# myshell-ai/OpenVoice

Measured on AMD Instinct MI355X. Metric: real_time_factor, higher is better.
Workload: dtype f32; 1 GPU; ToneColorConverter.convert path, 32 x 10 s @ 22.05 kHz per GPU (T=861 frames), fp32, calibrated random weights; batch_per_gpu=32, global_batch=32, parallelism=dp1 (utterance sharding, RCCL broadcast of src/tgt se)

## Files before the change

include/openvoice_amd.h:

```cpp
#ifndef OPENVOICE_AMD_H
#define OPENVOICE_AMD_H

#include <stddef.h>
#include <stdint.h>

#ifdef __cplusplus
extern "C" {
#endif

typedef void* ov_stream_t;

enum {
  OV_OK = 0,
  OV_E_BADARG = -1,
  OV_E_UNSUPPORTED = -2,
  OV_E_ALIGN = -3,
  OV_E_LAUNCH = -4
};

enum {
  OV_EPI_LINEAR = 0,
  OV_EPI_GATE = 1,
  OV_EPI_RESSKIP = 2,
  OV_EPI_COUPLE = 3,
// ... 309 lines not shown
  const float* bias;
  float* out;
  const float* res;
  const float* add;
  int64_t x_bstride, out_bstride, res_bstride, add_bstride;
  int32_t B, Cin, Cout, L;
  int32_t x_ld, out_ld;
  int32_t K, dil;
  int32_t nwg;
  int32_t frags;
  float in_slope;
  float scale;
  unsigned long long* dbg;
  const int32_t* col_limit;
  int32_t col_limit_scale;
  float out_slope;
} ov_conv1d_wino_params;
int ov_conv1d_wino_f32(const ov_conv1d_wino_params* p, ov_stream_t stream);
int ov_conv1d_wino_supported(int Cin, int Cout, int K, int dil);
int ov_conv1d_wino_chunk(int K, int Cout);
size_t ov_conv1d_wino_pack_size(int Cout, int Cin, int K);
int ov_conv1d_wino_pack_f32(const float* w, int Cout, int Cin, int K, float* dst);

int ov_version(void);
#define OV_ABI_VERSION 212
int ov_build_experiment(void);

#ifdef __cplusplus
}
#endif
#endif
```

openvoice_amd/_lib.py:

```python
import ctypes
import os

_HERE = os.path.dirname(os.path.abspath(__file__))
LIB_PATH = os.environ.get("OPENVOICE_AMD_LIB") or os.path.join(_HERE, "libopenvoice_amd.so")

OV_OK = 0
MIN_VERSION = 212
OV_ERRORS = {-1: "OV_E_BADARG", -2: "OV_E_UNSUPPORTED", -3: "OV_E_ALIGN", -4: "OV_E_LAUNCH"}

EPI_LINEAR, EPI_GATE, EPI_RESSKIP, EPI_COUPLE, EPI_POSTERIOR, EPI_CONVT, EPI_MAGNITUDE = range(7)
F_MASK_V = 1
F_OUT2_INIT = 2
F_CONVT_GROUPED = 4
F_NO_XCD_MAP = 8

_fp = ctypes.c_void_p
_i = ctypes.c_int
_i64 = ctypes.c_int64
LN_PRE_RELU, LN_POST_GELU = 1, 2


class ConvParams(ctypes.Structure):
    _fields_ = [
        ("x", _fp), ("w", _fp), ("bias", _fp), ("bias_b", _fp), ("out", _fp), ("res", _fp),
# ... 60 lines not shown
                ("nwg", ctypes.c_int32), ("frags", ctypes.c_int32),
                ("in_slope", ctypes.c_float), ("scale", ctypes.c_float), ("dbg", _fp),
                ("col_limit", _fp), ("col_limit_scale", ctypes.c_int32), ("out_slope", ctypes.c_float)]


class WnLayerParams(ctypes.Structure):
    _fields_ = [("x", _fp), ("out", _fp), ("skip", _fp), ("w_in", _fp), ("b_in", _fp), ("cond", _fp), ("w_rs", _fp),
                ("b_rs", _fp), ("mask", _fp),
                ("bstride", ctypes.c_int64), ("cond_bstride", ctypes.c_int64), ("mask_bstride", ctypes.c_int64),
                ("B", ctypes.c_int32), ("H", ctypes.c_int32), ("T", ctypes.c_int32), ("ld", ctypes.c_int32),
                ("K", ctypes.c_int32), ("first", ctypes.c_int32), ("last", ctypes.c_int32), ("width", ctypes.c_int32),
                ("ntile", ctypes.c_int32), ("row_split", ctypes.c_int32), ("dbg", _fp), ("acts", _fp)]


SIGNATURES = {
    "ov_version": (ctypes.c_int, []),
    "ov_build_experiment": (ctypes.c_int, []),
    "ov_conv1d_pack_size": (ctypes.c_size_t, [ctypes.c_int, ctypes.c_int, ctypes.c_int]),
    "ov_conv1d_pack_rows": (ctypes.c_int, [ctypes.c_int]),
    "ov_conv1d_pack_f32": (ctypes.c_int, [_fp, ctypes.c_int, ctypes.c_int, ctypes.c_int, _fp]),
    "ov_conv1d_f32": (ctypes.c_int, [ctypes.POINTER(ConvParams), _fp]),
    "ov_resblock_pair_f32": (ctypes.c_int, [ctypes.POINTER(RespairParams), _fp]),
    "ov_resblock_pair_supported": (ctypes.c_int, [_i, _i, _i]),
    "ov_wn_layer_f32": (ctypes.c_int, [ctypes.POINTER(WnLayerParams), _fp]),
    "ov_wn_layer_supported": (ctypes.c_int, [_i, _i]),
    "ov_wn_pack_size": (ctypes.c_size_t, [_i, _i, _i]),
    "ov_wn_pack_f32": (ctypes.c_int, [_fp, _i, _i, _i, _fp]),
    "ov_wn_layer_tile": (ctypes.c_int, [_i, _i, _i]),
    "ov_wn_layer_wino_f32": (ctypes.c_int, [ctypes.POINTER(WnLayerParams), _fp]),
    "ov_wn_layer_wino_tile": (ctypes.c_int, []),
    "ov_wn_wino_pack_size": (ctypes.c_size_t, [_i, _i, _i]),
    "ov_wn_wino_pack_f32": (ctypes.c_int, [_fp, _i, _i, _i, _fp]),
    "ov_conv_post_tanh_f32": (ctypes.c_int, [_fp, _fp, _fp, ctypes.c_int, ctypes.c_int, ctypes.c_int,
                                             ctypes.c_int, ctypes.c_float, _fp]),
    "ov_conv_post_tanh_limited_f32": (ctypes.c_int, [_fp, _fp, _fp, ctypes.c_int, ctypes.c_int, ctypes.c_int,
                                                     ctypes.c_int, ctypes.c_float, _fp, ctypes.c_int, _fp]),
    "ov_frame_limits_i32": (ctypes.c_int, [_fp, _fp, _i, _i, _i, _fp]),
    "ov_linear_f32": (ctypes.c_int, [_fp, _fp, _fp, _fp, ctypes.c_int, ctypes.c_int, ctypes.c_int, _fp]),
    "ov_sequence_mask_f32": (ctypes.c_int, [_fp, _fp, ctypes.c_int, ctypes.c_int, ctypes.c_int, _fp]),
    "ov_unpad_rows_f32": (ctypes.c_int, [_fp, _fp, ctypes.c_int, ctypes.c_int, ctypes.c_int, _fp]),
    "ov_polyphase_fir_f32": (ctypes.c_int, [_fp, _fp, _fp, ctypes.c_int64, ctypes.c_int64, _i, _i, _i, _fp]),
    "ov_polyphase_fir_rows_f32": (ctypes.c_int, [_fp, _i, _fp, _i64, _fp, _i64, _fp, _i64, _i64, _fp]),
    "ov_layernorm_freq_f32": (ctypes.c_int, [_fp, _fp, _fp, _fp, ctypes.c_int, ctypes.c_int, ctypes.c_int,
                                             ctypes.c_float, _fp]),
    "ov_conv2d_s2_relu_f32": (ctypes.c_int, [_fp, _fp, _fp, _fp, ctypes.c_int, ctypes.c_int, ctypes.c_int,
                                             ctypes.c_int, ctypes.c_int, _fp]),
# ... 83 lines not shown
    return _lib


def torch_op(name, *args):
    try:
        return getattr(torch_ops(), name)(*args)
    except RuntimeError as exc:
        if isinstance(exc, OvError):
            raise
        raise OvError(str(exc).split("\n")[0]) from None


def check(code, what):
    if code != OV_OK:
        raise OvError(f"{what} failed: {OV_ERRORS.get(code, code)}")


SHIM_PATH = os.path.join(_HERE, "libopenvoice_amd_torch.so")
_ops = None
VALUE_FUNCS = {"ov_version", "ov_build_experiment", "ov_conv1d_pack_size", "ov_conv1d_pack_rows", "ov_wn_pack_size",
               "ov_conv1d_bf16_pack_size", "ov_resblock_pair_supported", "ov_wn_layer_supported", "ov_wn_layer_tile",
               "ov_resblock_pair_bf16_supported", "ov_resblock_pair2_bf16_supported", "ov_conv1d_split3_pack_size",
               "ov_conv1d_split3_supported", "ov_conv1d_wino_supported", "ov_conv1d_wino_chunk", "ov_conv1d_wino_pack_size",
               "ov_wn_layer_wino_tile", "ov_wn_wino_pack_size"}


def binding():
    b = os.environ.get("OPENVOICE_AMD_BINDING", "ctypes" if os.environ.get("OPENVOICE_AMD_LIB") else "torch")
    if b not in ("torch", "ctypes"):
        raise OvError(f"OPENVOICE_AMD_BINDING={b!r}: expected 'torch' or 'ctypes'")
    return b


def use_torch_binding():
    return binding() == "torch"


def torch_ops():
    global _ops
    if _ops is None:
        import torch
        for path in (LIB_PATH, SHIM_PATH):
            if not os.path.exists(path):
                raise OvError(f"{path} not found: build the HIP extension first (python -c 'import __graft_entry__ "
                              f"as g; g.build()'); there is no CPU fallback (OPENVOICE_AMD_BINDING=ctypes needs only "
                              f"libopenvoice_amd.so)")
        torch.ops.load_library(SHIM_PATH)
# ... 49 lines not shown
```

openvoice_amd/csrc/torch_shim.cpp:

```cpp
#include <ATen/ATen.h>
#include <ATen/hip/impl/HIPGuardImplMasqueradingAsCUDA.h>
#include <c10/hip/HIPStream.h>
#include <torch/library.h>

#include <string>
#include <type_traits>

#include "openvoice_amd.h"

namespace {

const char* ov_strerror(int rc) {
  switch (rc) {
    case OV_E_BADARG: return "OV_E_BADARG";
    case OV_E_UNSUPPORTED: return "OV_E_UNSUPPORTED";
    case OV_E_ALIGN: return "OV_E_ALIGN";
    case OV_E_LAUNCH: return "OV_E_LAUNCH";
    default: return "unknown error";
  }
}

using OptTensor = c10::optional<at::Tensor>;

struct Ctx {
// ... 180 lines not shown
  DeviceScope scope(c);
  finish(ov_conv1d_f32(&p, c.stream()), "ov_conv1d_f32");
}

void resblock_pair_f32(const OptTensor& x, const OptTensor& w1, const OptTensor& b1, const OptTensor& w2,
                       const OptTensor& b2, const OptTensor& out, const OptTensor& add, const OptTensor& dbg,
                       const OptTensor& col_limit, at::IntArrayRef ip, at::ArrayRef<double> fp) {
  TORCH_CHECK(ip.size() == 11 && fp.size() == 2, "openvoice_amd::resblock_pair_f32: 11 integer and 2 float parameters");
  Ctx c{"resblock_pair_f32", false};
  ov_respair_params p{};
  p.x = sptr<float>(x, c, 0); p.w1 = sptr<float>(w1, c, 1); p.b1 = sptr<float>(b1, c, 2);
  p.w2 = sptr<float>(w2, c, 3); p.b2 = sptr<float>(b2, c, 4); p.out = sptr<float>(out, c, 5);
  p.add = sptr<float>(add, c, 6);
  p.dbg = sptr<unsigned long long>(dbg, c, 7);
  p.col_limit = sptr<int32_t>(col_limit, c, 8);
  p.B = (int32_t)ip[0]; p.C = (int32_t)ip[1]; p.L = (int32_t)ip[2]; p.ld = (int32_t)ip[3]; p.K = (int32_t)ip[4];
  p.dil = (int32_t)ip[5]; p.nwg = (int32_t)ip[6];
  p.x_bstride = ip[7]; p.out_bstride = ip[8]; p.add_bstride = ip[9]; p.col_limit_scale = (int32_t)ip[10];
  p.slope = (float)fp[0]; p.scale = (float)fp[1];
  DeviceScope scope(c);
  finish(ov_resblock_pair_f32(&p, c.stream()), "ov_resblock_pair_f32");
}

template <int (*FN)(const ov_wn_layer_params*, ov_stream_t)>
void wn_layer_any(const char* op, const char* entry, const OptTensor& x, const OptTensor& out, const OptTensor& skip,
                  const OptTensor& w_in, const OptTensor& b_in, const OptTensor& cond, const OptTensor& w_rs,
                  const OptTensor& b_rs, const OptTensor& mask, const OptTensor& dbg, const OptTensor& acts,
                  at::IntArrayRef ip) {
  TORCH_CHECK(ip.size() == 13, "openvoice_amd::", op, ": 13 integer parameters");
  Ctx c{op, false};
  ov_wn_layer_params p{};
  p.x = sptr<float>(x, c, 0); p.out = sptr<float>(out, c, 1); p.skip = sptr<float>(skip, c, 2);
  p.w_in = sptr<float>(w_in, c, 3); p.b_in = sptr<float>(b_in, c, 4); p.cond = sptr<float>(cond, c, 5, ip[11]);
  p.w_rs = sptr<float>(w_rs, c, 6); p.b_rs = sptr<float>(b_rs, c, 7); p.mask = sptr<float>(mask, c, 8);
  p.dbg = sptr<unsigned long long>(dbg, c, 9);
  p.acts = sptr<float>(acts, c, 10);
  p.B = (int32_t)ip[0]; p.H = (int32_t)ip[1]; p.T = (int32_t)ip[2]; p.ld = (int32_t)ip[3]; p.K = (int32_t)ip[4];
  p.first = (int32_t)ip[5]; p.last = (int32_t)ip[6]; p.width = (int32_t)ip[7];
  p.bstride = ip[8]; p.cond_bstride = ip[9]; p.mask_bstride = ip[10]; p.row_split = (int32_t)ip[12];
  DeviceScope scope(c);
  finish(FN(&p, c.stream()), entry);
}
void wn_layer_f32(const OptTensor& x, const OptTensor& out, const OptTensor& skip, const OptTensor& w_in,
                  const OptTensor& b_in, const OptTensor& cond, const OptTensor& w_rs, const OptTensor& b_rs,
                  const OptTensor& mask, const OptTensor& dbg, const OptTensor& acts, at::IntArrayRef ip) {
  wn_layer_any<&ov_wn_layer_f32>("wn_layer_f32", "ov_wn_layer_f32", x, out, skip, w_in, b_in, cond, w_rs, b_rs, mask, dbg, acts, ip);
// ... 77 lines not shown
                     at::ArrayRef<double> fp) {
  TORCH_CHECK(ip.size() == 15 && fp.size() == 3, "openvoice_amd::conv1d_wino_f32: 15 integer and 3 float parameters");
  Ctx c{"conv1d_wino_f32", false};
  ov_conv1d_wino_params p{};
  p.x = sptr<float>(x, c, 0); p.w = sptr<float>(w, c, 1); p.bias = sptr<float>(bias, c, 2);
  p.out = sptr<float>(out, c, 3); p.res = sptr<float>(res, c, 4); p.add = sptr<float>(add, c, 5);
  p.dbg = sptr<unsigned long long>(dbg, c, 6);
  p.col_limit = sptr<int32_t>(col_limit, c, 7); p.col_limit_scale = (int32_t)ip[14];
  p.B = (int32_t)ip[0]; p.Cin = (int32_t)ip[1]; p.Cout = (int32_t)ip[2]; p.L = (int32_t)ip[3];
  p.x_ld = (int32_t)ip[4]; p.out_ld = (int32_t)ip[5]; p.K = (int32_t)ip[6]; p.dil = (int32_t)ip[7]; p.nwg = (int32_t)ip[8];
  p.x_bstride = ip[9]; p.out_bstride = ip[10]; p.res_bstride = ip[11]; p.add_bstride = ip[12]; p.frags = (int32_t)ip[13];
  p.in_slope = (float)fp[0]; p.scale = (float)fp[1]; p.out_slope = (float)fp[2];
  DeviceScope scope(c);
  finish(ov_conv1d_wino_f32(&p, c.stream()), "ov_conv1d_wino_f32");
}

}

TORCH_LIBRARY(openvoice_amd, m) {
  m.def("conv1d_f32(Tensor? x, Tensor? w, Tensor? bias, Tensor(a!)? out, Tensor? res, Tensor? add, Tensor(b!)? out2, "
        "Tensor? mask, Tensor? bias_b, Tensor? col_limit, int[] ip, float[] fp) -> ()", &conv1d_f32);
  m.def("resblock_pair_f32(Tensor? x, Tensor? w1, Tensor? b1, Tensor? w2, Tensor? b2, Tensor(a!)? out, Tensor? add, "
        "Tensor(b!)? dbg, Tensor? col_limit, int[] ip, float[] fp) -> ()", &resblock_pair_f32);
  m.def("wn_layer_f32(Tensor? x, Tensor(a!)? out, Tensor(b!)? skip, Tensor? w_in, Tensor? b_in, Tensor? cond, Tensor? w_rs, "
        "Tensor? b_rs, Tensor? mask, Tensor(c!)? dbg, Tensor(d!)? acts, int[] ip) -> ()", &wn_layer_f32);
  m.def("wn_layer_wino_f32(Tensor? x, Tensor(a!)? out, Tensor(b!)? skip, Tensor? w_in, Tensor? b_in, Tensor? cond, Tensor? w_rs, "
        "Tensor? b_rs, Tensor? mask, Tensor(c!)? dbg, Tensor(d!)? acts, int[] ip) -> ()", &wn_layer_wino_f32);
  m.def("conv1d_bf16cl(Tensor? x, Tensor? w, Tensor? bias, Tensor(a!)? out, Tensor? res, Tensor? add, Tensor(b!)? dbg, "
        "int[] ip, float[] fp) -> ()", &conv1d_bf16cl);
  m.def("resblock_pair_bf16cl(Tensor? x, Tensor? w1, Tensor? b1, Tensor? w2, Tensor? b2, Tensor(a!)? out, Tensor? add, "
        "Tensor(b!)? dbg, int[] ip, float[] fp) -> ()", &resblock_pair_bf16cl);
  m.def("resblock_pair2_bf16cl(Tensor? x, Tensor? w1, Tensor? b1, Tensor? w2, Tensor? b2, Tensor(a!)? out, Tensor? add, "
        "Tensor(b!)? dbg, int[] ip, float[] fp) -> ()", &resblock_pair2_bf16cl);
  m.def("conv1d_split3(Tensor? x, Tensor? w, Tensor? bias, Tensor(a!)? out, Tensor? res, Tensor(b!)? dbg, "
        "Tensor? col_limit, int[] ip, float[] fp) -> ()", &conv1d_split3);
  m.def("conv1d_wino_f32(Tensor? x, Tensor? w, Tensor? bias, Tensor(a!)? out, Tensor? res, Tensor? add, Tensor(b!)? dbg, "
        "Tensor? col_limit, int[] ip, float[] fp) -> ()",
        &conv1d_wino_f32);
  bind_device<&ov_frame_hops_f32>(m, "frame_hops_f32");
  bind_device<&ov_frame_hops_windows_f32>(m, "frame_hops_windows_f32");
  bind_device<&ov_frame_hops_multi_f32>(m, "frame_hops_multi_f32");
  bind_device<&ov_carry_rows_f32>(m, "carry_rows_f32");
  bind_device<&ov_rows_f32_to_cl_bf16>(m, "rows_f32_to_cl_bf16");
  bind_device<&ov_cl_bf16_to_rows_f32>(m, "cl_bf16_to_rows_f32");
  bind_device<&ov_vad_frame_energy_f32>(m, "vad_frame_energy_f32");
  bind_device<&ov_vad_segments_i32>(m, "vad_segments_i32");
// ... 26 lines not shown
  bind_device<&ov_expand_prior_f32>(m, "expand_prior_f32");
  bind_device<&ov_conv_post_tanh_bf16>(m, "conv_post_tanh_bf16");
  bind_device<&ov_split3_from_f32>(m, "split3_from_f32");
  bind_device<&ov_split3_to_f32>(m, "split3_to_f32");
  bind_host<&ov_conv1d_pack_f32>(m, "conv1d_pack_f32");
  bind_host<&ov_wn_pack_f32>(m, "wn_pack_f32");
  bind_host<&ov_wn_wino_pack_f32>(m, "wn_wino_pack_f32");
  bind_value<&ov_wn_wino_pack_size>(m, "wn_wino_pack_size");
  bind_value<&ov_wn_layer_wino_tile>(m, "wn_layer_wino_tile");
  bind_host<&ov_conv1d_bf16_pack>(m, "conv1d_bf16_pack");
  bind_host<&ov_conv1d_bf16_pack16>(m, "conv1d_bf16_pack16");
  bind_host<&ov_conv1d_split3_pack>(m, "conv1d_split3_pack");
  bind_value<&ov_conv1d_split3_pack_size>(m, "conv1d_split3_pack_size");
  bind_value<&ov_conv1d_split3_supported>(m, "conv1d_split3_supported");
  bind_host<&ov_conv1d_wino_pack_f32>(m, "conv1d_wino_pack_f32");
  bind_value<&ov_conv1d_wino_pack_size>(m, "conv1d_wino_pack_size");
  bind_value<&ov_conv1d_wino_supported>(m, "conv1d_wino_supported");
  bind_value<&ov_conv1d_wino_chunk>(m, "conv1d_wino_chunk");
  bind_value<&ov_conv1d_pack_size>(m, "conv1d_pack_size");
  bind_value<&ov_conv1d_pack_rows>(m, "conv1d_pack_rows");
  bind_value<&ov_wn_pack_size>(m, "wn_pack_size");
  bind_value<&ov_conv1d_bf16_pack_size>(m, "conv1d_bf16_pack_size");
  bind_value<&ov_resblock_pair_supported>(m, "resblock_pair_supported");
  bind_value<&ov_wn_layer_supported>(m, "wn_layer_supported");
  bind_value<&ov_wn_layer_tile>(m, "wn_layer_tile");
  bind_value<&ov_resblock_pair_bf16_supported>(m, "resblock_pair_bf16_supported");
  bind_value<&ov_resblock_pair2_bf16_supported>(m, "resblock_pair2_bf16_supported");
  bind_value<&ov_version>(m, "version");
  bind_value<&ov_build_experiment>(m, "build_experiment");
}
```

openvoice_amd/engine.py:

```python
import ctypes
import os

import torch

from . import _lib
from . import noise as noise_mod
from ._lib import (ConvParams, EPI_CONVT, EPI_COUPLE, EPI_GATE, EPI_LINEAR, EPI_POSTERIOR, EPI_RESSKIP,
                   F_CONVT_GROUPED, F_MASK_V, F_OUT2_INIT)
from .params import ENC_Q_LAYERS, FLOW_LAYERS, N_FLOWS, REF_ENC_FILTERS, REF_ENC_GRU, effective_weight

GENERATOR_MARGIN = 16
LIMIT_MAX_BATCH = 256
LRELU_SLOPE = 0.1
FINAL_LRELU_SLOPE = 0.01


SUPPORTED_RESBLOCK_KERNELS = (3, 7, 11)
SUPPORTED_RESBLOCK_DILATIONS = (1, 3, 5)


def validate_config(cfg):
    def bad(field, value, why):
        raise _lib.OvError(f"config field {field!r} = {value!r} is not supported by the MI355X kernels: {why}")

# ... 189 lines not shown
    _lib.check(_lib.load().ov_conv1d_f32(ctypes.byref(p), stream), "ov_conv1d_f32")


def launch_pair(c1, c2, x, x_bs, out, out_bs, B, L, add=None, add_bs=0, scale=1.0, slope=LRELU_SLOPE, ld=0, nwg=0,
                dbg=None, col_limit=None, col_limit_scale=1):
    if _lib.use_torch_binding():
        _lib.torch_op("resblock_pair_f32", x, c1.w, c1.bias, c2.w, c2.bias, out, add, dbg, col_limit,
                      [B, c1.cin, L, ld, c1.K, c1.dil, nwg, x_bs, out_bs, add_bs, col_limit_scale], [slope, scale])
        return
    p = _lib.RespairParams()
    p.x, p.w1, p.b1, p.w2, p.b2 = _ptr(x), _ptr(c1.w), _ptr(c1.bias), _ptr(c2.w), _ptr(c2.bias)
    p.out = _ptr(out)
    p.add = _ptr(add) if add is not None else None
    p.x_bstride, p.out_bstride, p.add_bstride = x_bs, out_bs, add_bs
    p.B, p.C, p.L, p.ld, p.K, p.dil, p.nwg = B, c1.cin, L, ld, c1.K, c1.dil, nwg
    p.slope, p.scale = slope, scale
    p.dbg = ctypes.c_void_p(dbg.data_ptr()) if dbg is not None else None
    p.col_limit = ctypes.c_void_p(col_limit.data_ptr()) if col_limit is not None else None
    p.col_limit_scale = col_limit_scale
    stream = ctypes.c_void_p(torch.cuda.current_stream(x.device).cuda_stream)
    _lib.check(_lib.load().ov_resblock_pair_f32(ctypes.byref(p), stream), "ov_resblock_pair_f32")


_pair_supported = {}


def pair_supported(C, K, dil):
    key = (C, K, dil)
    if key not in _pair_supported:
        _pair_supported[key] = bool(_lib.call("ov_resblock_pair_supported", C, K, dil))
    return _pair_supported[key]


PAIR_POLICY = {(32, 3), (32, 7)}


def wino_policy(C, K, dil):
    return C >= 64 or dil == 1


WINO_MIN_ITEMS = 136

SPLIT_MIN_CHANNELS = 128


def _wino_mw(cout):
    return 4 if cout % 128 == 0 else (2 if cout % 64 == 0 else 1)


def wino_ncol(cout, dil):
    return (256 if dil == 1 else 4 * (64 // dil) * dil) * (4 // _wino_mw(cout))


def wino_items(cout, dil, B, L):
    ncol = wino_ncol(cout, dil)
    return B * ((L + ncol - 1) // ncol) * (cout // (32 * _wino_mw(cout)))


DIRECT_MIN_NCOL = 128


def conv_reach(family, K, dil=1):
    if family in ("direct", "pair", "split3"):
        r = (K - 1) // 2 * dil
        return r, r
    if family == "wino":
        from . import wino
        G = (K + 2) // 3
        pad = (K - 1) // 2 + wino.LEAD_TAPS[K]
        return (pad + 2) * dil, (3 * (G - 1) + 4 - pad) * dil
    raise ValueError(f"unknown conv family {family!r}")


def resblock_families(C, K, dils, B, L, use_winograd=True, fuse_pairs=True):
    from . import wino
    if fuse_pairs and L % 4 == 0 and all((C, K) in PAIR_POLICY and pair_supported(C, K, d) for d in dils):
        return [("pair", "pair")] * len(dils)
    fam = lambda d: ("wino" if use_winograd and L % 4 == 0 and wino.supported(C, C, K, d) and wino_policy(C, K, d)
                     and wino_items(C, d, B, L) >= WINO_MIN_ITEMS else "direct")
    return [(fam(d), fam(1)) for d in dils]


def limit_margin_frames(cfg, B, T, use_winograd=True, fuse_pairs=True):
    ch0, rates = cfg["upsample_initial_channel"], cfg["upsample_rates"]

    def chain_reach(i, k, dils):
        C, L = ch0 >> (i + 1), T
        for u in rates[:i + 1]:
            L *= u
        fams = resblock_families(C, k, dils, B, L, use_winograd, fuse_pairs)
        return sum(conv_reach(f1, k, d)[1] + conv_reach(f2, k, 1)[1] for (f1, f2), d in zip(fams, dils))

    return max(GENERATOR_MARGIN, generator_margin_frames(cfg), generator_margin_frames(cfg, chain_reach=chain_reach))


def wn_fused_row_order(hidden):
    assert hidden % 8 == 0
    idx = []
    for q in range(hidden // 8):
        for j in range(4):
# ... 232 lines not shown
        from . import wino
        kw = dict(in_slope=in_slope, out_slope=out_slope, scale=scale, res=res, res_bs=bs if res is not None else 0, add=add,
                  add_bs=bs if add is not None else 0, **lim)
        if self.profile is None:
            wino.launch_conv_wino(layer, x, bs, out, bs, B, L, **kw)
            return
        e0, e1 = torch.cuda.Event(enable_timing=True), torch.cuda.Event(enable_timing=True)
        e0.record()
        wino.launch_conv_wino(layer, x, bs, out, bs, B, L, **kw)
        e1.record()
        alg = 2.0 * layer.cout * layer.cin * layer.K * L * B
        self.profile.append(("mrf", alg, e0, e1, alg * wino.PRODUCTS_PER_TILE[layer.K] / (4.0 * layer.K)))

    def _pair(self, c1, c2, x, out, bs, B, L, add, scale, **lim):
        if self.profile is None:
            launch_pair(c1, c2, x, bs, out, bs, B, L, add=add, add_bs=bs, scale=scale, **lim)
            return
        e0, e1 = torch.cuda.Event(enable_timing=True), torch.cuda.Event(enable_timing=True)
        e0.record()
        launch_pair(c1, c2, x, bs, out, bs, B, L, add=add, add_bs=bs, scale=scale, **lim)
        e1.record()
        self.profile.append(("mrf", 2 * 2.0 * c1.rows * c1.cin * c1.K * L * B, e0, e1))

    def _linear(self, x2d, w, b):
        Bg, Kd = x2d.shape
        M = w.shape[0]
        y = torch.empty(Bg, M, dtype=torch.float32, device=self.device)
        _lib.call("ov_linear_f32", x2d, w, b, y, Bg, M, Kd)
        return y

    def _wn_cond(self, wn, g):
        if self.fuse_wn and wn.fused:
            return self._linear(g, wn.cond_w_fused, wn.cond_b_fused)
        return self._linear(g, wn.cond_w, wn.cond_b)

    def _workspace(self, B, T):
        key = (B, T)
        ws = self._ws.pop(key, None)
        if ws is not None:
            self._ws[key] = ws
        else:
            while self._ws and len(self._ws) >= max(1, int(self.resident_workspaces)):
                self._ws.pop(next(iter(self._ws)))
            dev, H, C = self.device, self.hidden, self.inter
            Tp = padded_frames(T)
            f = lambda *shape: torch.zeros(*shape, dtype=torch.float32, device=dev)
# ... 297 lines not shown
        concurrent = (self.chain_streams > 1 and nk > 1 and B <= self.chain_streams_max_batch and self.profile is None
                      and not (torch.cuda.is_current_stream_capturing() and len(ws.get("dec_extra", [])) < 2 * (nk - 1)))
        scratch = [(t1, ra)]
        if concurrent:
            extra = self._chain_scratch(ws, 2 * (nk - 1))
            scratch += [(extra[2 * j], extra[2 * j + 1]) for j in range(nk - 1)]

        def chain(j, pairs):
            t1_, ra_ = scratch[j if concurrent else 0]
            cur = u
            fams = resblock_families(ch, pairs[0][0].K, [c1.dil for c1, _ in pairs], B, L, self.use_winograd,
                                     self.fuse_pairs)
            fused = fams[0][0] == "pair"
            wn = self.wino_resblocks[i][j]
            for n, (c1, c2) in enumerate(pairs):
                last = n == len(pairs) - 1
                if last and concurrent and j > 0:
                    torch.cuda.current_stream(self.device).wait_event(done[j - 1])
                add = acc if (last and j > 0) else None
                scale = 1.0 / nk if (last and j == nk - 1) else 1.0
                if fused:
                    dst = acc if last else (t1_ if cur is ra_ else ra_)
                    self._pair(c1, c2, cur, dst, bs, B, L, add, scale, **lim(rate))
                else:
                    w1, w2 = (w if f == "wino" else None for w, f in zip(wn[n], fams[n]))
                    if w1 is not None:
                        self._wino(w1, cur, t1_, bs, B, L, out_slope=LRELU_SLOPE, **lim(rate))
                    else:
                        self._conv(c1, cur, 0, bs, t1_, 0, bs, B, L, in_slope=LRELU_SLOPE, tag="mrf", **lim(rate))
                    c2_slope = 1.0 if w1 is not None else LRELU_SLOPE
                    dst = acc if last else ra_
                    if w2 is not None:
                        self._wino(w2, t1_, dst, bs, B, L, res=cur, add=add, scale=scale, in_slope=c2_slope, **lim(rate))
                    else:
                        self._conv(c2, t1_, 0, bs, dst, 0, bs, B, L, in_slope=c2_slope, res=cur, res_bs=bs,
                                   add=add, add_bs=bs, scale=scale, tag="mrf", **lim(rate))
                cur = dst

        if not concurrent:
            for j, pairs in enumerate(self.resblocks[i]):
                chain(j, pairs)
        else:
            main = torch.cuda.current_stream(self.device)
            side = self._side_streams(nk)
            fork = torch.cuda.Event()
            fork.record(main)
# ... 311 lines not shown
```

Before: 3107 x real-time (audio s / wall s).

## Add fused Winograd resblock pair kernel for 64-channel K=3 convs

Adds a new kernel that runs both convolutions of a resblock pair (dilated conv and dil-1 conv) with Winograd F(4,3) on MFMA. The intermediate activation stays in LDS instead of going through global memory, and producer waves overlap loading and input transform with the MFMA waves. The engine picks this 'winopair' family for 64-channel, K=3 resblocks with enough work items, taking over from the separate wino/direct launches. This saves one kernel launch and a global round-trip per pair, but uses a lot of LDS per block and adds a complex warp-specialized schedule.

```diff
diff --git a/include/openvoice_amd.h b/include/openvoice_amd.h
--- a/include/openvoice_amd.h
+++ b/include/openvoice_amd.h
@@ -355,6 +355,11 @@
 size_t ov_conv1d_wino_pack_size(int Cout, int Cin, int K);
 int ov_conv1d_wino_pack_f32(const float* w, int Cout, int Cin, int K, float* dst);
 
+int ov_resblock_pair_wino_f32(const ov_respair_params* p, ov_stream_t stream);
+int ov_resblock_pair_wino_supported(int C, int K, int dil);
+int ov_resblock_pair_wino_block(int C, int dil);
+int ov_resblock_pair_wino_shift(int C, int dil);
+
 int ov_version(void);
 #define OV_ABI_VERSION 212
 int ov_build_experiment(void);
diff --git a/openvoice_amd/_lib.py b/openvoice_amd/_lib.py
--- a/openvoice_amd/_lib.py
+++ b/openvoice_amd/_lib.py
@@ -106,6 +106,10 @@
     "ov_conv1d_f32": (ctypes.c_int, [ctypes.POINTER(ConvParams), _fp]),
     "ov_resblock_pair_f32": (ctypes.c_int, [ctypes.POINTER(RespairParams), _fp]),
     "ov_resblock_pair_supported": (ctypes.c_int, [_i, _i, _i]),
+    "ov_resblock_pair_wino_f32": (ctypes.c_int, [ctypes.POINTER(RespairParams), _fp]),
+    "ov_resblock_pair_wino_supported": (ctypes.c_int, [_i, _i, _i]),
+    "ov_resblock_pair_wino_block": (ctypes.c_int, [_i, _i]),
+    "ov_resblock_pair_wino_shift": (ctypes.c_int, [_i, _i]),
     "ov_wn_layer_f32": (ctypes.c_int, [ctypes.POINTER(WnLayerParams), _fp]),
     "ov_wn_layer_supported": (ctypes.c_int, [_i, _i]),
     "ov_wn_pack_size": (ctypes.c_size_t, [_i, _i, _i]),
@@ -235,7 +239,9 @@
                "ov_conv1d_bf16_pack_size", "ov_resblock_pair_supported", "ov_wn_layer_supported", "ov_wn_layer_tile",
                "ov_resblock_pair_bf16_supported", "ov_resblock_pair2_bf16_supported", "ov_conv1d_split3_pack_size",
                "ov_conv1d_split3_supported", "ov_conv1d_wino_supported", "ov_conv1d_wino_chunk", "ov_conv1d_wino_pack_size",
-               "ov_wn_layer_wino_tile", "ov_wn_wino_pack_size"}
+               "ov_wn_layer_wino_tile", "ov_wn_wino_pack_size",
+               "ov_resblock_pair_wino_supported", "ov_resblock_pair_wino_block",
+               "ov_resblock_pair_wino_shift"}
 
 
 def binding():
diff --git a/openvoice_amd/csrc/conv1d_wino_pair.h b/openvoice_amd/csrc/conv1d_wino_pair.h
--- /dev/null
+++ b/openvoice_amd/csrc/conv1d_wino_pair.h
@@ -0,0 +1,471 @@
+#pragma once
+#include "conv1d_wino.h"
+
+namespace ovkw {
+
+template <int DIL>
+struct PairGeo {
+  static constexpr int C = 64, CI = 8, NCH = C / CI, NT = 64;
+  using Gd = GeoD<3, DIL == 1 ? 3 : DIL, 2>;
+  static constexpr int TC = DIL == 1 ? 256 : Gd::NCOL;
+  static constexpr int SH = DIL == 1 ? 0 : 4 * DIL - 4;
+  static constexpr int W = (TC - 8) / (4 * DIL) * (4 * DIL);
+  static_assert((SH + 4) % (4 * DIL) == 0 && W % (4 * DIL) == 0 && W + 8 <= TC, "tile grid of conv 1");
+  static constexpr int ORG = DIL == 1 ? 8 : Gd::PADA;
+  static constexpr int RW = DIL == 1 ? TC + 16 : Gd::RW;
+  static constexpr int TW = 272;
+};
+
+template <int DIL>
+__global__ __launch_bounds__(512, 2) void wino_pair_kernel(const ov_respair_params p) {
+  using PG = PairGeo<DIL>;
+  using Ge = Geo<3>;
+  using Gd = typename PG::Gd;
+  constexpr int CI = PG::CI, NCH = PG::NCH, NT = PG::NT, RW = PG::RW, TW = PG::TW, W = PG::W, ORG = PG::ORG, SH = PG::SH;
+  constexpr int NSTEP = CI / 2, NPAIR = NSTEP / 2, NPR = CI / 2, RW4 = RW / 4;
+  constexpr int NITEM = NPR * RW4, RAWBUF = CI * RW, VBUF = CI * NT * 6;
+  constexpr int PER = 2 * NCH;
+  __shared__ __attribute__((aligned(16))) float raw[2 * RAWBUF];
+  __shared__ __attribute__((aligned(16))) float Vs[2 * VBUF];
+  __shared__ __attribute__((aligned(16))) float tt[PG::C * TW];
+  __shared__ __attribute__((aligned(16))) float bias_s[2 * PG::C];
+  __shared__ int lim_pref[ovk::LIMIT_MAX_BATCH + 1];
+
+  const int tid = threadIdx.x;
+  const int lane = tid & 63;
+  const int wave = __builtin_amdgcn_readfirstlane(tid >> 6);
+  const int L = p.L;
+  const int nblk = (L + SH + W - 1) / W;
+  int total = nblk * p.B;
+  const bool limited = p.col_limit != nullptr;
+  if (limited) {
+    if (wave == 0) {
+      int carry = 0;
+      for (int base = 0; base < p.B; base += 64) {
+        const int bb = base + lane;
+        int nb = 0;
+        if (bb < p.B) {
+          long long c = (long long)p.col_limit[bb] * p.col_limit_scale;
+          c = c < 0 ? 0 : (c > L ? L : c);
+          nb = c > 0 ? ((int)c + SH + W - 1) / W : 0;
+        }
+        int sc = nb;
+#pragma unroll
+        for (int d = 1; d < 64; d <<= 1) {
+          const int v = __shfl_up(sc, d, 64);
+          if (lane >= d) sc += v;
+        }
+        if (bb < p.B) lim_pref[bb + 1] = carry + sc;
+        carry += __shfl(sc, 63, 64);
+      }
+      if (lane == 0) lim_pref[0] = 0;
+    }
+    __syncthreads();
+    total = __builtin_amdgcn_readfirstlane(lim_pref[p.B]);
+  }
+  auto decode = [&](int g, int& ub, int& ublk) {
+    if (!limited) {
+      ub = g / nblk;
+      ublk = g - ub * nblk;
+      return;
+    }
+    int lo = 0, hi = p.B;
+    while (hi - lo > 1) {
+      const int mid = (lo + hi) >> 1;
+      if (__builtin_amdgcn_readfirstlane(lim_pref[mid]) <= g) lo = mid; else hi = mid;
+    }
+    ub = lo;
+    ublk = g - __builtin_amdgcn_readfirstlane(lim_pref[lo]);
+  };
+  int wid0 = blockIdx.x, wend = total, wstride = gridDim.x;
+  if ((gridDim.x & 7u) == 0) {
+    const int xcd = blockIdx.x & 7;
+    const int lo = (int)(((long long)xcd * total) >> 3);
+    wend = (int)(((long long)(xcd + 1) * total) >> 3);
+    wid0 = lo + (int)(blockIdx.x >> 3);
+    wstride = gridDim.x >> 3;
+  }
+  if (wid0 >= wend) return;
+  const int nitems = (wend - wid0 + wstride - 1) / wstride;
+  const int npos = nitems * PER;
+  if (tid < PG::C) bias_s[tid] = p.b1[tid];
+  else if (tid < 2 * PG::C) bias_s[tid] = p.b2[tid - PG::C];
+  const uint32_t LD = (uint32_t)p.ld;
+
+  if (wave >= 4) {
+    __builtin_amdgcn_s_setprio(3);
+    const float slope = p.slope;
+    const int hl = (wave - 4) * 64 + lane;
+    constexpr int NLOAD = (NITEM + 255) / 256;
+    f32x4 sa[2][NLOAD], sb[2][NLOAD];
+    uint32_t sbyte[NLOAD];
+    int scol[NLOAD];
+    int nval[2][NLOAD];
+    uint32_t hasbits = 0;
+    bool edge[2] = {false, false};
+#pragma unroll
+    for (int i = 0; i < NLOAD; ++i) {
+      const int idx = i * 256 + hl;
+      const int pr = idx / RW4, c4 = idx - pr * RW4;
+      const bool has = idx < NITEM;
+      hasbits |= (has ? 1u : 0u) << i;
+      scol[i] = 4 * c4;
+      sbyte[i] = has ? 4u * (2u * (uint32_t)pr * LD + 4u * (uint32_t)c4) : 0u;
+      nval[0][i] = nval[1][i] = 0;
+    }
+    const uint32_t raw_lds = lds_addr(raw) + 32u * (uint32_t)hl;
+    const uint32_t v_lds = lds_addr(Vs);
+    int lwid = wid0, lchunk = 0, lb, lblk;
+    decode(lwid, lb, lblk);
+
+    auto issue_loads = [&](auto setc) {
+      constexpr int S = decltype(setc)::value;
+      const int tb = lblk * W - SH - 4 - ORG;
+      const float* __restrict__ xrow = p.x + (int64_t)lb * p.x_bstride + (int64_t)(lchunk * CI) * LD;
+      edge[S] = !(tb >= 0 && tb + RW <= L);
+      if (!edge[S]) {
+        const char* b0 = reinterpret_cast<const char*>(xrow + tb);
+        const char* b1 = reinterpret_cast<const char*>(xrow + tb + LD);
+#pragma unroll
+        for (int i = 0; i < NLOAD; ++i) {
+          sa[S][i] = *reinterpret_cast<const f32x4*>(b0 + sbyte[i]);
+          sb[S][i] = *reinterpret_cast<const f32x4*>(b1 + sbyte[i]);
+        }
+      } else {
+        const char* b0 = reinterpret_cast<const char*>(xrow);
+        const char* b1 = reinterpret_cast<const char*>(xrow + LD);
+#pragma unroll
+        for (int i = 0; i < NLOAD; ++i) {
+          const int t = tb + scol[i];
+          int nv = L - t;
+          nv = (((hasbits >> i) & 1u) && t >= 0 && nv > 0) ? (nv > 4 ? 4 : nv) : 0;
+          const uint32_t off = nv > 0 ? sbyte[i] + 4u * (uint32_t)tb : 0u;
+          nval[S][i] = nv;
+          sa[S][i] = *reinterpret_cast<const f32x4*>(b0 + off);
+          sb[S][i] = *reinterpret_cast<const f32x4*>(b1 + off);
+        }
+      }
+      if (++lchunk == NCH) {
+        lchunk = 0;
+        lwid += wstride;
+        if (lwid < wend) decode(lwid, lb, lblk);
+      }
+    };
+    auto act2 = [&](f32x2 v) {
+      const f32x2 sv = v * f32x2{slope, slope};
+      f32x2 r;
+      asm("v_max_f32 %0, %1, %2" : "=v"(r[0]) : "v"(v[0]), "v"(sv[0]));
+      asm("v_max_f32 %0, %1, %2" : "=v"(r[1]) : "v"(v[1]), "v"(sv[1]));
+      return r;
+    };
+    auto write_raw = [&](int buf, auto setc) {
+      constexpr int S = decltype(setc)::value;
+      const uint32_t base = raw_lds + (uint32_t)buf * (RAWBUF * 4);
+#pragma unroll
+      for (int i = 0; i < NLOAD; ++i) {
+        if ((hasbits >> i) & 1u) {
+          f32x2 a01 = {sa[S][i][0], sa[S][i][1]}, a23 = {sa[S][i][2], sa[S][i][3]};
+          f32x2 b01 = {sb[S][i][0], sb[S][i][1]}, b23 = {sb[S][i][2], sb[S][i][3]};
+          if (slope != 1.f) {
+            a01 = act2(a01); a23 = act2(a23); b01 = act2(b01); b23 = act2(b23);
+          }
+          if (edge[S]) {
+            const int nv = nval[S][i];
+            if (nv < 1) { a01[0] = 0.f; b01[0] = 0.f; }
+            if (nv < 2) { a01[1] = 0.f; b01[1] = 0.f; }
+            if (nv < 3) { a23[0] = 0.f; b23[0] = 0.f; }
+            if (nv < 4) { a23[1] = 0.f; b23[1] = 0.f; }
+          }
+          const uint32_t ad = base + (uint32_t)i * (256 * 32);
+          asm volatile("ds_write2_b32 %0, %1, %2 offset1:1" ::"v"(ad), "v"(a01[0]), "v"(b01[0]) : "memory");
+          asm volatile("ds_write2_b32 %0, %1, %2 offset0:2 offset1:3" ::"v"(ad), "v"(a01[1]), "v"(b01[1]) : "memory");
+          asm volatile("ds_write2_b32 %0, %1, %2 offset0:4 offset1:5" ::"v"(ad), "v"(a23[0]), "v"(b23[0]) : "memory");
+          asm volatile("ds_write2_b32 %0, %1, %2 offset0:6 offset1:7" ::"v"(ad), "v"(a23[1]), "v"(b23[1]) : "memory");
+        }
+      }
+    };
+    static_assert(NPR * NT == 256, "one round of helper lanes per chunk");
+    const int tile = hl & (NT - 1), pr = hl / NT;
+    uint32_t tsrc_x;
+    if constexpr (DIL == 1) {
+      tsrc_x = 8u * (uint32_t)(pr * RW + Ge::WSTART + 4 * tile);
+    } else {
+      const int rc0 = tile / Gd::J, rc = rc0 < DIL ? rc0 : 0, jt = rc0 < DIL ? tile - rc0 * Gd::J : 0;
+      tsrc_x = 8u * (uint32_t)(pr * RW + (Gd::PADA - Gd::PADD) + rc + 4 * DIL * jt);
+    }
+    const uint32_t tsrc_t = 8u * (uint32_t)(pr * TW + Ge::WSTART + 4 * tile);
+    uint32_t vadr[2][6];
+#pragma unroll
+    for (int bf = 0; bf < 2; ++bf)
+#pragma unroll
+      for (int q = 0; q < 6; ++q) vadr[bf][q] = v_lds + (uint32_t)bf * (VBUF * 4) + 24u * (uint32_t)(2 * pr * NT + tile) + 4u * q;
+    auto transform = [&](const char* src, auto widec, auto bufc) {
+      constexpr bool WIDE = decltype(widec)::value;
+      constexpr int buf = decltype(bufc)::value;
+      constexpr int NWIN = WIDE ? 4 * Ge::NB128 : Gd::NV;
+      f32x2 win[NWIN];
+      if constexpr (WIDE) {
+#pragma unroll
+        for (int q = 0; q < 2 * Ge::NB128; ++q) {
+          const f32x4 v = *reinterpret_cast<const f32x4*>(src + 16 * q);
+          win[2 * q] = f32x2{v[0], v[1]};
+          win[2 * q + 1] = f32x2{v[2], v[3]};
+        }
+      } else {
+#pragma unroll
+        for (int u = 0; u < Gd::NV; ++u) win[u] = *reinterpret_cast<const f32x2*>(src + 8 * DIL * u);
+      }
+      constexpr int o = WIDE ? Ge::OFF0 - Ge::WSTART : 0;
+      const f32x2 d0 = win[o], d1 = win[o + 1], d2 = win[o + 2], d3 = win[o + 3], d4 = win[o + 4], d5 = win[o + 5];
+      const f32x2 c4 = {4.f, 4.f}, m4 = {-4.f, -4.f}, m5 = {-5.f, -5.f}, c2 = {2.f, 2.f}, m2 = {-2.f, -2.f};
+      const f32x2 t1 = __builtin_elementwise_fma(m4, d2, d4), t2 = __builtin_elementwise_fma(m4, d1, d3);
+      const f32x2 t3 = d4 - d2, t4 = d3 - d1;
+      const f32x2 v0 = __builtin_elementwise_fma(c4, d0, __builtin_elementwise_fma(m5, d2, d4));
+      const f32x2 v1 = t1 + t2;
+      const f32x2 v2 = t1 - t2;
+      const f32x2 v3 = __builtin_elementwise_fma(c2, t4, t3);
+      const f32x2 v4 = __builtin_elementwise_fma(m2, t4, t3);
+      const f32x2 v5 = __builtin_elementwise_fma(c4, d1, __builtin_elementwise_fma(m5, d3, d5));
+      constexpr int OB = NT * 24 / 256;
+      static_assert((NT * 24) % 256 == 0, "channel record distance in 256-byte units");
+      lds_write2st64_b32<0, OB>(vadr[buf][0], v0[0], v0[1]);
+      lds_write2st64_b32<0, OB>(vadr[buf][1], v1[0], v1[1]);
+      lds_write2st64_b32<0, OB>(vadr[buf][2], v2[0], v2[1]);
+      lds_write2st64_b32<0, OB>(vadr[buf][3], v3[0], v3[1]);
+      lds_write2st64_b32<0, OB>(vadr[buf][4], v4[0], v4[1]);
+      lds_write2st64_b32<0, OB>(vadr[buf][5], v5[0], v5[1]);
+    };
+    using WX = std::integral_constant<bool, DIL == 1>;
+    auto transform_x = [&](auto bufc) {
+      constexpr int buf = decltype(bufc)::value;
+      transform(reinterpret_cast<const char*>(raw) + buf * (RAWBUF * 4) + tsrc_x, WX{}, bufc);
+    };
+    auto transform_t = [&](int chunk, auto bufc) {
+      transform(reinterpret_cast<const char*>(tt) + (uint32_t)chunk * (NPR * TW * 8) + tsrc_t, std::true_type{}, bufc);
+    };
+    auto is_x = [&](int pos) { return pos < npos && (pos & (PER - 1)) < NCH; };
+    static_assert((PER & (PER - 1)) == 0 && NCH >= 4, "stream arithmetic");
+
+    using S0 = std::integral_constant<int, 0>;
+    using S1 = std::integral_constant<int, 1>;
+    issue_loads(S0{});
+    write_raw(0, S0{});
+    issue_loads(S1{});
+    lds_barrier();
+    transform_x(S0{});
+    write_raw(1, S1{});
+    issue_loads(S0{});
+    lds_barrier();
+    auto period = [&](int i, auto par) {
+      constexpr int P = decltype(par)::value;
+      using Q = std::integral_constant<int, 1 - P>;
+      if (is_x(i + 3)) issue_loads(Q{});
+      const int nq = (i + 1) & (PER - 1);
+      const bool nlive = i + 1 < npos;
+      if (nlive) {
+        if (nq < NCH) transform_x(Q{});
+        else if (nq > NCH) transform_t(nq - NCH, Q{});
+      }
+      if (is_x(i + 2)) write_raw(P, par);
+      lds_barrier();
+      if (nlive && nq == NCH) {
+        lds_barrier();
+        transform_t(0, Q{});
+        lds_barrier();
+      }
+    };
+    for (int i = 0; i < npos; i += 2) {
+      period(i, S0{});
+      period(i + 1, S1{});
+    }
+    return;
+  }
+
+  const int half = lane >> 5, n = lane & 31;
+  const int wrow = wave & 1, wfr = wave >> 1;
+  const int tile = 32 * wfr + n;
+  const f32x4* __restrict__ w1 = reinterpret_cast<const f32x4*>(p.w1);
+  const f32x4* __restrict__ w2 = reinterpret_cast<const f32x4*>(p.w2);
+  const uint32_t rec0 = (uint32_t)wrow * (uint32_t)(NCH * NPAIR * 3);
+  int wid = wid0, b, blk;
+  decode(wid, b, blk);
+  f32x4 a_cur[3], a_nxt[3];
+#pragma unroll
+  for (int j = 0; j < 3; ++j) a_cur[j] = w1[(size_t)(rec0 + j) * 64 + lane];
+  const int voffB = (half * NT + tile) * 6;
+  const float oslope = p.slope;
+  const float scale = p.scale;
+
+  __syncthreads();
+  __syncthreads();
+  int it = 0;
+  while (true) {
+    const int s0 = blk * W - SH;
+    f32x16 acc[6];
+#pragma unroll 1
+    for (int ph = 0; ph < 2; ++ph) {
+      const f32x4* __restrict__ wbase = ph == 0 ? w1 : w2;
+      uint32_t rec = rec0;
+#pragma unroll
+      for (int q = 0; q < 6; ++q)
+#pragma unroll
+        for (int r = 0; r < 16; ++r) acc[q][r] = 0.f;
+#pragma unroll
+      for (int i = 0; i < 4; ++i) {
+        const f32x4 bq = *reinterpret_cast<const f32x4*>(bias_s + ph * PG::C + wrow * 32 + 4 * half + 8 * i);
+        acc[1][4 * i] = bq[0]; acc[1][4 * i + 1] = bq[1]; acc[1][4 * i + 2] = bq[2]; acc[1][4 * i + 3] = bq[3];
+      }
+      f32x2 bq[3];
+#pragma unroll
+      for (int qq = 0; qq < 3; ++qq) bq[qq] = *reinterpret_cast<const f32x2*>(Vs + (it & 1) * VBUF + voffB + 2 * qq);
+      for (int chunk = 0; chunk < NCH; ++chunk, ++it) {
+        const float* vb = Vs + (it & 1) * VBUF + voffB;
+        const float* vbn = Vs + ((it + 1) & 1) * VBUF + voffB;
+        const bool more_chunks = chunk + 1 < NCH;
+#pragma unroll
+        for (int s = 0; s < NSTEP; ++s) {
+          const int s2 = s & 1;
+          if (s == NSTEP - 1) lds_barrier();
+          if (s2 == 0) {
+            rec += 3;
+#pragma unroll
+            for (int j = 0; j < 3; ++j) a_nxt[j] = wbase[(size_t)(rec + j) * 64 + lane];
+          }
+#pragma unroll
+          for (int qq = 0; qq < 3; ++qq) {
+            __builtin_amdgcn_sched_barrier(0);
+#pragma unroll
+            for (int t = 0; t < 2; ++t) {
+              const int q = 2 * qq + t, e = s2 * 6 + q;
+              acc[q] = __builtin_amdgcn_mfma_f32_32x32x2f32(a_cur[e >> 2][e & 3], bq[qq][t], acc[q], 0, 0, 0);
+            }
+            __builtin_amdgcn_sched_barrier(0);
+            if (s + 1 < NSTEP || more_chunks)
+              bq[qq] = *reinterpret_cast<const f32x2*>((s + 1 < NSTEP ? vb + (s + 1) * (2 * NT * 6) : vbn) + 2 * qq);
+          }
+          if (s2 == 1) {
+#pragma unroll
+            for (int j = 0; j < 3; ++j) a_cur[j] = a_nxt[j];
+          }
+        }
+      }
+      auto at4 = [&](int r) {
+        const float y0 = acc[0][r], y1 = acc[1][r], y2 = acc[2][r], y3 = acc[3][r], y4 = acc[4][r], y5 = acc[5][r];
+        const float s1 = y1 + y2, d1 = y1 - y2, s2 = y3 + y4, d2 = y3 - y4;
+        f32x4 o;
+        o[0] = (y0 + s1) + s2;
+        o[1] = __builtin_fmaf(2.f, d2, d1);
+        o[2] = __builtin_fmaf(4.f, s2, s1);
+        o[3] = __builtin_fmaf(8.f, d2, d1) + y5;
+        return o;
+      };
+      if (ph == 0) {
+#pragma unroll
+        for (int j = 0; j < 3; ++j) a_cur[j] = w2[(size_t)(rec0 + j) * 64 + lane];
+        int tix[4];
+        if constexpr (DIL == 1) {
+#pragma unroll
+          for (int e = 0; e < 4; ++e) tix[e] = 4 + 4 * tile + e;
+        } else {
+          const int rc0 = tile / Gd::J, jt = tile - rc0 * Gd::J;
+#pragma unroll
+          for (int e = 0; e < 4; ++e) tix[e] = rc0 < DIL ? 4 + rc0 + DIL * (4 * jt + e) : -1;
+        }
+        bool inside[4];
+#pragma unroll
+        for (int e = 0; e < 4; ++e) {
+          const int col = s0 - 8 + tix[e];
+          inside[e] = col >= 0 && col < L;
+        }
+#pragma unroll
+        for (int i = 0; i < 4; ++i)
+#pragma unroll
+          for (int jp = 0; jp < 2; ++jp) {
+            f32x4 oa = at4(4 * i + 2 * jp), ob = at4(4 * i + 2 * jp + 1);
+#pragma unroll
+            for (int e = 0; e < 4; ++e) {
+              oa[e] = inside[e] ? ovk::lrelu(oa[e], oslope) : 0.f;
+              ob[e] = inside[e] ? ovk::lrelu(ob[e], oslope) : 0.f;
+            }
+            float* row = tt + (16 * wrow + 4 * i + 2 * half + jp) * (2 * TW);
+            if constexpr (DIL == 1) {
+              *reinterpret_cast<f32x4*>(row + 2 * tix[0]) = f32x4{oa[0], ob[0], oa[1], ob[1]};
+              *reinterpret_cast<f32x4*>(row + 2 * tix[0] + 4) = f32x4{oa[2], ob[2], oa[3], ob[3]};
+            } else {
+              if (tix[0] >= 0) {
+#pragma unroll
+                for (int e = 0; e < 4; ++e) *reinterpret_cast<f32x2*>(row + 2 * tix[e]) = f32x2{oa[e], ob[e]};
+              }
+            }
+          }
+        lds_barrier();
+        lds_barrier();
+      } else {
+        const int nwid = wid + wstride;
+        const bool more = nwid < wend;
+        const int ob_ = b;
+        if (more) {
+#pragma unroll
+          for (int j = 0; j < 3; ++j) a_cur[j] = w1[(size_t)(rec0 + j) * 64 + lane];
+          wid = nwid;
+          decode(wid, b, blk);
+        }
+        float* outb = p.out + (int64_t)ob_ * p.out_bstride;
+        const float* resb = p.x + (int64_t)ob_ * p.x_bstride;
+        const float* addb = p.add ? p.add + (int64_t)ob_ * p.add_bstride : nullptr;
+        const int col = s0 + 4 * tile;
+        const bool colok = 4 * tile < W && col >= 0 && col < L;
+        const int nv = colok ? L - col : 0;
+        const uint32_t voff = 4u * (uint32_t)half * LD + (colok ? (uint32_t)col : 0u);
+        const size_t mrow = (size_t)wrow * 32u;
+        auto run = [&](auto has_add) {
+          constexpr bool HA = decltype(has_add)::value;
+          constexpr int DEPTH = HA ? 4 : 8;
+          f32x4 rv[DEPTH], av[HA ? DEPTH : 1];
+          auto load = [&](int g) {
+            const size_t rowb = (mrow + (size_t)((g & 3) + 8 * (g >> 2))) * LD;
+            rv[g % DEPTH] = *reinterpret_cast<const f32x4*>(resb + rowb + voff);
+            if constexpr (HA) av[g % DEPTH] = *reinterpret_cast<const f32x4*>(addb + rowb + voff);
+          };
+#pragma unroll
+          for (int g = 0; g < DEPTH - 1; ++g) load(g);
+#pragma unroll
+          for (int g = 0; g < 16; ++g) {
+            if (g + DEPTH - 1 < 16) load(g + DEPTH - 1);
+            f32x4 o = at4(g);
+            o += rv[g % DEPTH];
+            if constexpr (HA) o += av[g % DEPTH];
+            o *= scale;
+            float* dst = outb + (mrow + (size_t)((g & 3) + 8 * (g >> 2))) * LD + voff;
+            if (nv >= 4) {
+              *reinterpret_cast<f32x4*>(dst) = o;
+            } else if (nv > 0) {
+              dst[0] = o[0];
+              if (nv > 1) dst[1] = o[1];
+              if (nv > 2) dst[2] = o[2];
+            }
+          }
+        };
+        if (addb) run(std::true_type{});
+        else run(std::false_type{});
+        if (!more) return;
+      }
+    }
+  }
+}
+
+template <int DIL>
+int wino_pair_launch(const ov_respair_params* p, hipStream_t stream) {
+  constexpr int W = PairGeo<DIL>::W, SH = PairGeo<DIL>::SH;
+  const long total = (long)((p->L + SH + W - 1) / W) * p->B;
+  auto kernel = wino_pair_kernel<DIL>;
+  static std::atomic<int> slot_cache[ovk::OV_MAX_DEVICES];
+  const int slots = ovk::resident_workgroups(reinterpret_cast<const void*>(kernel), 512, slot_cache);
+  long nwg = p->nwg > 0 ? p->nwg : slots;
+  if (nwg > total) nwg = total;
+  if (nwg >= 8) nwg = (nwg + 7) / 8 * 8;
+  hipLaunchKernelGGL(kernel, dim3((unsigned)nwg), dim3(512), 0, stream, *p);
+  return hipGetLastError() == hipSuccess ? OV_OK : OV_E_LAUNCH;
+}
+
+}
diff --git a/openvoice_amd/csrc/conv1d_wino_pair.hip b/openvoice_amd/csrc/conv1d_wino_pair.hip
--- /dev/null
+++ b/openvoice_amd/csrc/conv1d_wino_pair.hip
@@ -0,0 +1,50 @@
+#include "conv1d_wino_pair.h"
+
+using namespace ovkw;
+
+extern "C" {
+
+int ov_resblock_pair_wino_supported(int C, int K, int dil) {
+  return (C == PairGeo<1>::C && K == 3 && (dil == 1 || dil == 3 || dil == 5)) ? 1 : 0;
+}
+
+int ov_resblock_pair_wino_block(int C, int dil) {
+  if (!ov_resblock_pair_wino_supported(C, 3, dil)) return 0;
+  return dil == 1 ? PairGeo<1>::W : (dil == 3 ? PairGeo<3>::W : PairGeo<5>::W);
+}
+
+int ov_resblock_pair_wino_shift(int C, int dil) {
+  if (!ov_resblock_pair_wino_supported(C, 3, dil)) return 0;
+  return dil == 1 ? PairGeo<1>::SH : (dil == 3 ? PairGeo<3>::SH : PairGeo<5>::SH);
+}
+
+int ov_resblock_pair_wino_f32(const ov_respair_params* pin, ov_stream_t stream) {
+  if (!pin) return OV_E_BADARG;
+  ov_respair_params q = *pin;
+  if (!q.x || !q.w1 || !q.b1 || !q.w2 || !q.b2 || !q.out) return OV_E_BADARG;
+  if (q.B <= 0 || q.L <= 0 || q.nwg < 0) return OV_E_BADARG;
+  if (q.col_limit && (q.col_limit_scale <= 0 || (reinterpret_cast<uintptr_t>(q.col_limit) & 3))) return OV_E_BADARG;
+  if (q.col_limit && q.B > ovk::LIMIT_MAX_BATCH) q.col_limit = nullptr;
+  if (q.ld == 0) q.ld = q.L;
+  if (q.ld < q.L) return OV_E_BADARG;
+  if (!ov_resblock_pair_wino_supported(q.C, q.K, q.dil)) return OV_E_UNSUPPORTED;
+  if (!(q.slope > 0.f && q.slope <= 1.f)) return OV_E_UNSUPPORTED;
+  if (q.out == q.x) return OV_E_BADARG;
+  auto mis = [](const void* ptr) { return (reinterpret_cast<uintptr_t>(ptr) & 15) != 0; };
+  if (mis(q.x) || mis(q.w1) || mis(q.w2) || mis(q.out) || (q.add && mis(q.add)) || (q.ld & 3) || (q.x_bstride & 3) ||
+      (q.out_bstride & 3) || (q.add && (q.add_bstride & 3)))
+    return OV_E_ALIGN;
+  if ((int64_t)q.C * q.ld >= (1LL << 28)) return OV_E_BADARG;
+  if (q.B > 1 && (q.x_bstride < (int64_t)q.C * q.ld || q.out_bstride < (int64_t)q.C * q.ld ||
+                  (q.add && q.add_bstride < (int64_t)q.C * q.ld)))
+    return OV_E_BADARG;
+  hipStream_t st = static_cast<hipStream_t>(stream);
+  switch (q.dil) {
+    case 1: return wino_pair_launch<1>(&q, st);
+    case 3: return wino_pair_launch<3>(&q, st);
+    case 5: return wino_pair_launch<5>(&q, st);
+  }
+  return OV_E_UNSUPPORTED;
+}
+
+}
diff --git a/openvoice_amd/csrc/torch_shim.cpp b/openvoice_amd/csrc/torch_shim.cpp
--- a/openvoice_amd/csrc/torch_shim.cpp
+++ b/openvoice_amd/csrc/torch_shim.cpp
@@ -226,6 +226,25 @@
   finish(ov_resblock_pair_f32(&p, c.stream()), "ov_resblock_pair_f32");
 }
 
+void resblock_pair_wino_f32(const OptTensor& x, const OptTensor& w1, const OptTensor& b1, const OptTensor& w2,
+                            const OptTensor& b2, const OptTensor& out, const OptTensor& add, const OptTensor& dbg,
+                            const OptTensor& col_limit, at::IntArrayRef ip, at::ArrayRef<double> fp) {
+  TORCH_CHECK(ip.size() == 11 && fp.size() == 2, "openvoice_amd::resblock_pair_wino_f32: 11 integer and 2 float parameters");
+  Ctx c{"resblock_pair_wino_f32", false};
+  ov_respair_params p{};
+  p.x = sptr<float>(x, c, 0); p.w1 = sptr<float>(w1, c, 1); p.b1 = sptr<float>(b1, c, 2);
+  p.w2 = sptr<float>(w2, c, 3); p.b2 = sptr<float>(b2, c, 4); p.out = sptr<float>(out, c, 5);
+  p.add = sptr<float>(add, c, 6);
+  p.dbg = sptr<unsigned long long>(dbg, c, 7);
+  p.col_limit = sptr<int32_t>(col_limit, c, 8);
+  p.B = (int32_t)ip[0]; p.C = (int32_t)ip[1]; p.L = (int32_t)ip[2]; p.ld = (int32_t)ip[3]; p.K = (int32_t)ip[4];
+  p.dil = (int32_t)ip[5]; p.nwg = (int32_t)ip[6];
+  p.x_bstride = ip[7]; p.out_bstride = ip[8]; p.add_bstride = ip[9]; p.col_limit_scale = (int32_t)ip[10];
+  p.slope = (float)fp[0]; p.scale = (float)fp[1];
+  DeviceScope scope(c);
+  finish(ov_resblock_pair_wino_f32(&p, c.stream()), "ov_resblock_pair_wino_f32");
+}
+
 template <int (*FN)(const ov_wn_layer_params*, ov_stream_t)>
 void wn_layer_any(const char* op, const char* entry, const OptTensor& x, const OptTensor& out, const OptTensor& skip,
                   const OptTensor& w_in, const OptTensor& b_in, const OptTensor& cond, const OptTensor& w_rs,
@@ -349,6 +368,8 @@
         "Tensor? mask, Tensor? bias_b, Tensor? col_limit, int[] ip, float[] fp) -> ()", &conv1d_f32);
   m.def("resblock_pair_f32(Tensor? x, Tensor? w1, Tensor? b1, Tensor? w2, Tensor? b2, Tensor(a!)? out, Tensor? add, "
         "Tensor(b!)? dbg, Tensor? col_limit, int[] ip, float[] fp) -> ()", &resblock_pair_f32);
+  m.def("resblock_pair_wino_f32(Tensor? x, Tensor? w1, Tensor? b1, Tensor? w2, Tensor? b2, Tensor(a!)? out, Tensor? add, "
+        "Tensor(b!)? dbg, Tensor? col_limit, int[] ip, float[] fp) -> ()", &resblock_pair_wino_f32);
   m.def("wn_layer_f32(Tensor? x, Tensor(a!)? out, Tensor(b!)? skip, Tensor? w_in, Tensor? b_in, Tensor? cond, Tensor? w_rs, "
         "Tensor? b_rs, Tensor? mask, Tensor(c!)? dbg, Tensor(d!)? acts, int[] ip) -> ()", &wn_layer_f32);
   m.def("wn_layer_wino_f32(Tensor? x, Tensor(a!)? out, Tensor(b!)? skip, Tensor? w_in, Tensor? b_in, Tensor? cond, Tensor? w_rs, "
@@ -421,6 +442,9 @@
   bind_value<&ov_wn_pack_size>(m, "wn_pack_size");
   bind_value<&ov_conv1d_bf16_pack_size>(m, "conv1d_bf16_pack_size");
   bind_value<&ov_resblock_pair_supported>(m, "resblock_pair_supported");
+  bind_value<&ov_resblock_pair_wino_supported>(m, "resblock_pair_wino_supported");
+  bind_value<&ov_resblock_pair_wino_block>(m, "resblock_pair_wino_block");
+  bind_value<&ov_resblock_pair_wino_shift>(m, "resblock_pair_wino_shift");
   bind_value<&ov_wn_layer_supported>(m, "wn_layer_supported");
   bind_value<&ov_wn_layer_tile>(m, "wn_layer_tile");
   bind_value<&ov_resblock_pair_bf16_supported>(m, "resblock_pair_bf16_supported");
diff --git a/openvoice_amd/engine.py b/openvoice_amd/engine.py
--- a/openvoice_amd/engine.py
+++ b/openvoice_amd/engine.py
@@ -235,6 +235,25 @@
     _lib.check(_lib.load().ov_resblock_pair_f32(ctypes.byref(p), stream), "ov_resblock_pair_f32")
 
 
+def launch_pair_wino(w1, w2, x, x_bs, out, out_bs, B, L, add=None, add_bs=0, scale=1.0, slope=LRELU_SLOPE, ld=0, nwg=0,
+                     col_limit=None, col_limit_scale=1):
+    ip = [B, w1.cin, L, ld, w1.K, w1.dil, nwg, x_bs, out_bs, add_bs, col_limit_scale]
+    if _lib.use_torch_binding():
+        _lib.torch_op("resblock_pair_wino_f32", x, w1.w, w1.bias, w2.w, w2.bias, out, add, None, col_limit, ip, [slope, scale])
+        return
+    p = _lib.RespairParams()
+    p.x, p.w1, p.b1, p.w2, p.b2 = _ptr(x), _ptr(w1.w), _ptr(w1.bias), _ptr(w2.w), _ptr(w2.bias)
+    p.out = _ptr(out)
+    p.add = _ptr(add) if add is not None else None
+    p.x_bstride, p.out_bstride, p.add_bstride = x_bs, out_bs, add_bs
+    p.B, p.C, p.L, p.ld, p.K, p.dil, p.nwg = B, w1.cin, L, ld, w1.K, w1.dil, nwg
+    p.slope, p.scale = slope, scale
+    p.col_limit = ctypes.c_void_p(col_limit.data_ptr()) if col_limit is not None else None
+    p.col_limit_scale = col_limit_scale
+    stream = ctypes.c_void_p(torch.cuda.current_stream(x.device).cuda_stream)
+    _lib.check(_lib.load().ov_resblock_pair_wino_f32(ctypes.byref(p), stream), "ov_resblock_pair_wino_f32")
+
+
 _pair_supported = {}
 
 
@@ -254,6 +273,18 @@
 
 WINO_MIN_ITEMS = 136
 
+WINO_PAIR_POLICY = {(64, 1), (64, 3), (64, 5)}
+
+
+def wino_pair_block(C, dil):
+    return _lib.call("ov_resblock_pair_wino_block", C, dil)
+
+
+def wino_pair_items(C, dil, B, L):
+    w = wino_pair_block(C, dil)
+    return B * ((L + _lib.call("ov_resblock_pair_wino_shift", C, dil) + w - 1) // w) if w else 0
+
+
 SPLIT_MIN_CHANNELS = 128
 
 
@@ -277,7 +308,7 @@
     if family in ("direct", "pair", "split3"):
         r = (K - 1) // 2 * dil
         return r, r
-    if family == "wino":
+    if family in ("wino", "winopair"):
         from . import wino
         G = (K + 2) // 3
         pad = (K - 1) // 2 + wino.LEAD_TAPS[K]
@@ -289,6 +320,9 @@
     from . import wino
     if fuse_pairs and L % 4 == 0 and all((C, K) in PAIR_POLICY and pair_supported(C, K, d) for d in dils):
         return [("pair", "pair")] * len(dils)
+    if use_winograd and fuse_pairs and K == 3 and L % 4 == 0 and all(
+            (C, d) in WINO_PAIR_POLICY and wino_pair_items(C, d, B, L) >= WINO_MIN_ITEMS for d in dils):
+        return [("winopair", "winopair")] * len(dils)
     fam = lambda d: ("wino" if use_winograd and L % 4 == 0 and wino.supported(C, C, K, d) and wino_policy(C, K, d)
                      and wino_items(C, d, B, L) >= WINO_MIN_ITEMS else "direct")
     return [(fam(d), fam(1)) for d in dils]
@@ -567,6 +601,18 @@
         e1.record()
         self.profile.append(("mrf", 2 * 2.0 * c1.rows * c1.cin * c1.K * L * B, e0, e1))
 
+    def _pair_wino(self, w1, w2, x, out, bs, B, L, add, scale, **lim):
+        from . import wino
+        if self.profile is None:
+            launch_pair_wino(w1, w2, x, bs, out, bs, B, L, add=add, add_bs=bs if add is not None else 0, scale=scale, **lim)
+            return
+        e0, e1 = torch.cuda.Event(enable_timing=True), torch.cuda.Event(enable_timing=True)
+        e0.record()
+        launch_pair_wino(w1, w2, x, bs, out, bs, B, L, add=add, add_bs=bs if add is not None else 0, scale=scale, **lim)
+        e1.record()
+        alg = 2 * 2.0 * w1.cout * w1.cin * w1.K * L * B
+        self.profile.append(("mrf", alg, e0, e1, alg * wino.PRODUCTS_PER_TILE[w1.K] / (4.0 * w1.K)))
+
     def _linear(self, x2d, w, b):
         Bg, Kd = x2d.shape
         M = w.shape[0]
@@ -910,6 +956,9 @@
                 if fused:
                     dst = acc if last else (t1_ if cur is ra_ else ra_)
                     self._pair(c1, c2, cur, dst, bs, B, L, add, scale, **lim(rate))
+                elif fams[n][0] == "winopair":
+                    dst = acc if last else (t1_ if cur is ra_ else ra_)
+                    self._pair_wino(wn[n][0], wn[n][1], cur, dst, bs, B, L, add, scale, **lim(rate))
                 else:
                     w1, w2 = (w if f == "wino" else None for w, f in zip(wn[n], fams[n]))
                     if w1 is not None:
```

Result: no change. 3122 x real-time (audio s / wall s) (median of 6 runs) (+0.5%).
